# aelmiger/LINE-MOD-Pipeline

Hardware: AMD Instinct MI355X
Metric: detections/sec (higher is better)
Workload: dtype u8

## Files before the change

line-mod-pipeline_amd/csrc/lm_common.h:

```cpp
#pragma once
#include <stdint.h>

typedef uint8_t u8;
typedef uint16_t u16;
typedef uint32_t u32;
typedef uint64_t u64;

#define LM_SCAN_CHUNK 1008
#define LM_SCAN4_CHUNK 1016
#define LM_SCAN_FPAD 8
#define LM_SCANL_LDS_BYTES 163840
#define LM_SCANL_IMAGE_MAX 153600
#define LM_SCANL_TABLE_BYTES 2048
#define LM_SCANL_POS_BITS 15
#define LM_SORT_CAP 4096
#define LM_SORT_CHUNK 1024
#define LM_INLINE_MATCHES 2048
#define LM_DROPPED 0xFFFFFFFFu

#define PD_STRIP 16
#define CB_ROWS 2
#define CBS_STRIP 16
#define MX_WAVE_BYTES 128
#define CVT_ROWS 4
#define CG_STRIP 16
#define CT_W 32
#define CT_H 8
#define DT_W 64
#define DT_H 8
#define DM_ROWS 4
#ifndef DM_ROWS_BATCH
#define DM_ROWS_BATCH 16
#endif
#define LMK_MAX_LOADS 8

struct LmPhaseGrid { u32 nb[4]; int g[4]; };

struct LmLevelGeom {
    int w, h;
    int T;
    int W, H;
    int spread_only;
    int nibble;
    u32 wh;
    u32 ori_stride;
    u32 plane_ori;
    u32 mod_stride;
// ... 42 lines not shown
```

line-mod-pipeline_amd/csrc/lm_detector.hip:

```cpp
#include "lm_detector_impl.h"
#include "lm_median_counts.h"

namespace lmd {

thread_local std::string g_err;
int fail(int code, const std::string& msg) { g_err = msg; return code; }

bool any_lane_busy(const lm_detector* d) {
    for (const lm_detector::Lane& ln : d->lanes) if (ln.busy) return true;
    return false;
}

void free_device_bank(lm_detector* d) {
    for (auto* b : {&d->d_item_t, &d->d_item_chunk, &d->d_scan_off, &d->d_off1, &d->d_offn, &d->d_offs3, &d->d_offl, &d->d_offsl, &d->d_litem}) b->reset();
    for (auto* b : {&d->d_scan_P, &d->d_scan_n, &d->d_t_global, &d->d_t_class}) b->reset();
    d->items1.clear();
    for (int l = 0; l < LM_MAX_LEVELS; ++l) { d->d_ref_meta[l].reset(); d->d_ref_feat[l].reset(); }
}

int ensure_device(lm_detector* d) {
    if (d->dev_ready) {
        HIP_TRY(hipSetDevice(d->cfg.device));
        return LM_OK;
    }
// ... 102 lines not shown
    }
    d->luts_dirty = false;
    return LM_OK;
}

int ensure_bank(lm_detector* d) {
    if (!d->bank_dirty) return LM_OK;
    HIP_TRY(hipDeviceSynchronize());
    free_device_bank(d);
    std::string err;
    if (!lmh::build_device_bank(d->bank, d->cfg, d->geom, d->hb, d->scan_list_order, err)) return fail(LM_ERR_INVALID, err);
    HIP_TRY(upload_vec(d->d_item_t, d->hb.item_t));
    HIP_TRY(upload_vec(d->d_item_chunk, d->hb.item_chunk));
    HIP_TRY(upload_vec(d->d_scan_off, d->hb.scan_off));
    HIP_TRY(upload_vec(d->d_scan_P, d->hb.scan_P));
    HIP_TRY(upload_vec(d->d_scan_n, d->hb.scan_n));
    if (d->hb.fpad1) {
        HIP_TRY(upload_vec(d->d_off1, d->hb.off1));
        HIP_TRY(upload_vec(d->d_offn, d->hb.offn));
        HIP_TRY(upload_vec(d->d_offs3, d->hb.offs3));
    }
    if (d->hb.lds_ok) {
        HIP_TRY(upload_vec(d->d_offl, d->hb.offl));
        HIP_TRY(upload_vec(d->d_offsl, d->hb.offsl));
        HIP_TRY(upload_vec(d->d_litem, d->hb.lrec));
    }
    HIP_TRY(upload_vec(d->d_t_global, d->hb.t_global));
    HIP_TRY(upload_vec(d->d_t_class, d->hb.t_class));
    for (int l = 0; l + 1 < d->cfg.pyramid_levels; ++l) {
        HIP_TRY(upload_vec(d->d_ref_meta[l], d->hb.ref_meta[l]));
        HIP_TRY(upload_vec(d->d_ref_feat[l], d->hb.ref_feat[l]));
    }
    d->bank_dirty = false;
    return LM_OK;
}

int check_slots(lm_detector* d, int first, int n) {
    if (first < 0 || n < 0 || first + n > (int)d->slots.size()) return fail(LM_ERR_INVALID, "slot out of range");
    return LM_OK;
}

bool normal_lut_onehot(lm_detector* d) {
    if (d->lut_onehot < 0) {
        d->lut_onehot = 1;
        for (int i = 0; i < 8000; ++i) { const u8 v = d->normal_lut[i]; if (v & (v - 1)) { d->lut_onehot = 0; break; } }
    }
    return d->lut_onehot != 0;
}

int refuse_checked_slots(const lm_detector* d, int first, int n) {
    if (d->cc_inflight && d->cc_pending && first <= d->cc_hi && d->cc_lo < first + n) return fail(LM_ERR_INVALID, "slot is read by a colour check in flight: call lm_color_check_end first");
    if (d->dc_inflight && d->dc_pending && first <= d->dc_hi && d->dc_lo < first + n) return fail(LM_ERR_INVALID, "slot is read by depth counts in flight: call lm_depth_counts_end first");
    const int icp_slot = d->icp_slot.load();
    if (icp_slot >= first && icp_slot < first + n) return fail(LM_ERR_INVALID, "slot is read by an ICP refinement in flight");
    return LM_OK;
}

lmh::ScanInputs scan_inputs(const lm_detector* d, const lm_detector::Lane& ln) {
    const LmLevelGeom& g = d->geom[d->cfg.pyramid_levels - 1];
    lmh::ScanInputs in;
    in.form = d->scan_form; in.M = d->cfg.num_modalities;
    in.nibble = g.nibble != 0; in.planes = g.plane_ori != 0; in.lds_fits = lmh::lds_image_fits(g, in.M);
    in.bank_built = !d->bank_dirty;
    in.scanl_bank = d->hb.lds_ok && d->d_litem; in.scanl_device = d->scanl_lds;
    in.fpad1 = d->hb.fpad1; in.items1_by_L = d->hb.items1_by_L; in.items4 = (long long)d->hb.item_t.size();
    in.frame_stride = d->frame_stride; in.arena_bytes = g.arena_bytes;
// ... 246 lines not shown

static int refuse_scan(lmh::ScanPlan::Kind k) {
    if (k == lmh::ScanPlan::Mixed)
        return fail(LM_ERR_INVALID, "the slots were prepared by calls of different scan forms (some keep only the spread byte of the scanned level): match them apart or upload again");
    return fail(LM_ERR_HIP, "the slots keep only the spread byte of the scanned level and the bit-plane scan could not be set up for them: upload the frames again");
}

static bool ensure_surv_queue(lm_detector* d, lm_detector::Lane& ln) {
    DevBuf<unsigned long long>& q = ln.d_surv;
    if (!q) {
        if (q.alloc(16 + (size_t)d->surv_cap) != hipSuccess) (void)hipGetLastError();
        else if (hipMemsetAsync(q, 0, 16 * sizeof(unsigned long long), ln.stream) != hipSuccess) { q.reset(); (void)hipGetLastError(); }
        ln.surv_set = 0;
    }
    return q != nullptr;
}

static lmh::MatchInputs match_inputs(const lm_detector* d, const lm_detector::Lane& ln, int first, ItemRange r, int nslots, int variant) {
    const int L = d->cfg.pyramid_levels;
    const LmLevelGeom& g = d->geom[L - 1];
    lmh::MatchInputs in;
    in.scan = scan_inputs(d, ln);
    in.layouts = slot_layouts(d, first, nslots); in.nslots = nslots;
    in.n_items = r.n;
    in.n_litems = d->hb.lds_ok ? d->hb.lbegin[(size_t)r.t_hi] - d->hb.lbegin[(size_t)r.t_lo] : 0;
    in.T = g.T; in.wh = g.wh; in.ori_stride = g.ori_stride; in.nibble = g.nibble != 0;
    in.M = d->cfg.num_modalities; in.L = L;
    for (int l = 0; l < L; ++l) in.level_W[l] = d->geom[l].W;
    in.miss_delta = d->miss_delta;
    in.have_plan = ln.plan != nullptr; in.plan_stride_cap = d->plan_stride_cap;
    in.variant = variant;
    in.sort_split_mode = d->sort_split_mode; in.sort_long_score = d->sort_long_score;
    return in;
}

int make_scan_args(lm_detector* d, lm_detector::Lane& ln, int first, ItemRange r, int nslots, int variant, lmh::MatchPlan* plan, LmScanArgs* out) {
    const int L = d->cfg.pyramid_levels;
    const LmLevelGeom& g = d->geom[L - 1];
    lmh::MatchInputs in = match_inputs(d, ln, first, r, nslots, variant);
    const lm_detector::Items1* it = nullptr;
    if (const int L1 = lmh::match_scan1_lanes(in))
        if (ensure_items1(d, L1, &it) == LM_OK) {
            in.items1_L = L1; in.n_items1 = it->begin[(size_t)r.t_hi] - it->begin[(size_t)r.t_lo];
            in.have_queue = ensure_surv_queue(d, ln);
        }
    lmh::MatchPlan& p = *plan;
    lmh::plan_match(in, p);
    if (p.kind == lmh::ScanPlan::Mixed || p.kind == lmh::ScanPlan::NoBitPlaneForm) return refuse_scan(p.kind);
    LmScanArgs& a = *out;
    a = LmScanArgs();
    a.lm = d->lm(first, L - 1); a.lm_slot_stride = d->frame_stride;
    a.item_t = d->d_item_t; a.item_chunk = d->d_item_chunk; a.item_lo = r.lo; a.n_items = p.n_items;
    a.nibble = g.nibble; a.M = d->cfg.num_modalities; a.fpad = d->hb.fpad; a.W = g.W; a.T = g.T;
    a.scan_off = d->d_scan_off; a.scan_P = d->d_scan_P; a.scan_n = d->d_scan_n;
    a.raw_thr_by_n = ln.d_raw_thr;
    a.hdr = reinterpret_cast<LmDevHeader*>(d->aux(first, d->off_hdr));
    a.cand = reinterpret_cast<LmCand*>(d->aux(first, d->off_cand));
    a.aux_slot_stride = d->aux_stride; a.cand_cap = d->max_cand;
    a.stat = d->scan_stats ? d->d_scan_stat : nullptr;
    a.wgs_per_slot = p.wgs_per_slot; a.nslots = nslots;
    a.L1 = p.L1; a.G1 = p.G1; a.L1_rcp16 = p.L1_rcp16; a.delta_rcp16 = p.delta_rcp16; a.no_exact = p.no_exact; a.exact_spread = p.exact_spread ? 1 : 0;
    a.R = p.R; a.pb = p.pb; a.planes_off = p.planes_off; a.tbl_bytes = p.tbl_bytes; a.queue_cap = p.queue_cap; a.dbg = p.dbg;
    if (p.kind != lmh::ScanPlan::Scan4) { a.fpad1 = d->hb.fpad1; a.offs3 = d->d_offs3; a.resp_tab = d->d_resp_tab; }
    if (p.kind == lmh::ScanPlan::ScanL) {
        a.lds_form = 1;
        a.offl = d->d_offl; a.offsl = d->d_offsl; a.litem = d->d_litem; a.litem_lo = d->hb.lbegin[(size_t)r.t_lo]; a.n_litems = in.n_litems;
        a.mod_stride = g.mod_stride; a.plane_ori = g.plane_ori;
    } else if (p.kind == lmh::ScanPlan::Scan1) {
        a.off1 = d->d_off1; a.offn = d->d_offn;
        a.item_t = it->d_t; a.item_chunk = it->d_chunk; a.item_lo = it->begin[(size_t)r.t_lo];
        a.surv = p.queue ? ln.d_surv : nullptr; a.surv_cap = d->surv_cap; a.surv_set = ln.surv_set;
    }
    return LM_OK;
}

void launch_scan(lm_detector::Lane& ln, const lmh::MatchPlan& plan, LmScanArgs& a) {
    lmk_scan_run(ln.stream, plan, a, ln.d_surv);
    if (!plan.flip_surv_set) return;
    ln.surv_set ^= 1;
    a.surv_set = ln.surv_set;
}

static LmRefineArgs make_refine_args(lm_detector* d, const lm_detector::Lane& ln, int first, int n, int level, float threshold, const lmh::MatchPlan& p) {
    LmRefineArgs a;
    a.lm = d->lm(first, level); a.lm_slot_stride = d->frame_stride;
    a.g = d->geom[level];
    a.M = d->cfg.num_modalities;
    a.meta = d->d_ref_meta[level]; a.feats = d->d_ref_feat[level];
    a.sim_lut = d->d_sim_lut;
    a.hdr = reinterpret_cast<LmDevHeader*>(d->aux(first, d->off_hdr));
    a.cand = reinterpret_cast<LmCand*>(d->aux(first, d->off_cand));
    a.keys = reinterpret_cast<u64*>(d->aux(first, d->off_keys));
    a.aux_slot_stride = d->aux_stride;
    a.cand_cap = d->max_cand; a.match_cap = d->max_match;
    a.threshold = threshold;
    a.t_global = d->d_t_global; a.t_class = d->d_t_class;
    a.plan = p.refine_plan ? ln.plan : nullptr; a.plan_cap = p.plan_cap;
    a.blocks_per_slot = p.blocks_per_slot; a.nslots = n;
// ... 679 lines not shown
```

line-mod-pipeline_amd/csrc/lm_detector_impl.h:

```cpp
#pragma once
#include <hip/hip_runtime.h>

#include <algorithm>
#include <climits>
#include <cmath>
#include <cstdio>
#include <cstdlib>
#include <cstring>
#include <string>
#include <vector>
#include <memory>
#include <mutex>
#include <atomic>

#include "../../include/linemod_hip.h"
#include "lm_common.h"
#include "lm_extract.h"
#include <thread>

#include "lm_host.h"
#include "lm_yaml.h"
#include "lm_kernels.h"
#include "lm_comm.h"
#include "lm_own.h"
// ... 42 lines not shown
struct IcpState;
struct GenState;
struct EvalState;

}
using namespace lmd;

struct lm_detector {
    ~lm_detector();
    lm_config cfg;
    LmLevelGeom geom[LM_MAX_LEVELS];
    int lw[LM_MAX_LEVELS], lh[LM_MAX_LEVELS];
    u8 sim_lut[256];
    u8 normal_lut[8000];
    int lut_onehot = -1;
    bool normal_lut_substitute = true;
    lmh::Bank bank;

    bool dev_ready = false;
    bool dev_begun = false;
    struct Gather {
        DevBuf<int> d_cnt; DevBuf<LmOutMatch> d_rec;
        DevBuf<int> d_all_cnt; DevBuf<LmOutMatch> d_all_rec;
        PinnedBuf<int> h_all_cnt; PinnedBuf<LmOutMatch> h_all_rec;
        bool active = false;
        u32 cap_lane = 0;
    };
    struct Lane {
        Stream stream;
        Event ev[6];
        DevBuf<int> d_raw_thr;
        PinnedBuf<int> h_raw_thr;
        float raw_thr_for = -1.0f;
        bool created = false, busy = false, timed = false;
        Event ev_done;
        Event blocking_ev;
        Event mask_done;
        int first = 0, n = 0;
        std::vector<int> classes;
        unsigned long long waited_seq[LM_NCOPY] = {};
        DevBuf<unsigned long long> d_surv;
        int surv_set = 0;
        u32* plan = nullptr;
        Gather gather;
        std::unique_ptr<LmComm> comm;
    };
    Lane lanes[LM_NLANES];
    Stream copy_stream[LM_NCOPY];
    unsigned long long up_seq_next[LM_NCOPY], up_seq_done[LM_NCOPY];
    int n_copy_streams = LM_NCOPY;
    int stage_chunks = 1;
    std::vector<Slot> slots;
    PinnedBuf<LmIngestDesc> h_ingest;
    DevBuf<LmIngestDesc> d_ingest;
    Event ev_ingest_src;
    bool reg_on = false, reg_rays_dirty = false;
    lm_registration_desc reg = {};
    std::vector<float> reg_rays;
    DevBuf<float> d_reg_rays;
    DevBuf<u32> d_reg_z[LM_NCOPY];
    bool rect_on = false, rect_map_dirty = false;
    lm_rectification_desc rect = {};
    std::vector<int32_t> rect_map;
    DevBuf<int32_t> d_rect_map;
    DevBuf<u8> frame_arena;
    size_t frame_stride = 0;
// ... 18 lines not shown
    int comm_recs_per_frame = 0;
    DevBuf<double> d_red;
    int batch_phases = 2;
    int scan_list_order = 3;
    int sort_split_mode = 2;
    int sort_long_score = 0;
    int work_weight_by_pixels = 1;
    int phase_max_slots = 15;
    DevBuf<u8> aux_arena;
    size_t aux_stride = 0;
    size_t off_hdr = 0, off_cand = 0, off_keys = 0, off_out = 0;
    PinnedBuf<u8> host_blocks;
    size_t host_stride = 0;
    DevBuf<u32> d_plan;
    int plan_stride_cap = 0;
    DevBuf<u64> d_resp_tab;
    int miss_delta = 1;
    DevBuf<u32> d_sim_lut;
    DevBuf<u8> d_normal_lut;
    bool luts_dirty = true;
    bool bank_dirty = true;
    lmh::DeviceBankHost hb;
    DevBuf<u32> d_item_t, d_item_chunk;
    DevBuf<u32> d_scan_off; DevBuf<int> d_scan_P, d_scan_n;
    DevBuf<int> d_t_global, d_t_class;
    DevBuf<u32> d_off1, d_offn;
    struct Items1 { int L = 0; DevBuf<u32> d_t, d_chunk; std::vector<int> begin; };
    std::vector<Items1> items1;
    int scan_form = 0;
    float scan1_min_threshold = 50.0f;
    long long cnt_scan1_launches = 0; int last_scan1_lanes = 0;
    DevBuf<u32> d_offs3;
    DevBuf<u32> d_offl, d_offsl, d_litem;
    DevBuf<unsigned long long> d_refine_stat;
    int scanl_min_slots = 24;
    int scanl_R = 0;
    bool scanl_lds = false;
    u32 surv_cap = 1u << 20;
    DevBuf<LmRefMeta> d_ref_meta[LM_MAX_LEVELS];
    DevBuf<LmRefFeat> d_ref_feat[LM_MAX_LEVELS];
    DevBuf<u8> d_scratch;
    u32 max_cand = 0, max_match = 0;
    int scan_variant = 0;
    bool scan_stats = false;
    DevBuf<unsigned long long> d_scan_stat;
    bool profiling = false;
    double prof_us[4] = {0, 0, 0, 0};
    double prof_scan_bytes = 0;
    long long prof_launches = 0, prof_frames = 0;
    long long prof_exch_fallbacks = 0;
    double prof_exch_us = 0; long long prof_exch_launches = 0;
    long long cnt_preprocess_frames = 0, cnt_scan_launches = 0, cnt_refine_launches = 0, cnt_sort_launches = 0;

    u8* bgr(int slot, int l) const { return frame_arena + (size_t)slot * frame_stride + off_bgr[l]; }
    u16* depth(int slot) const { return reinterpret_cast<u16*>(frame_arena + (size_t)slot * frame_stride + off_depth); }
    u8* quant(int slot, int l, int m) const { return frame_arena + (size_t)slot * frame_stride + off_quant[l][m]; }
    u8* lm(int slot, int l) const { return frame_arena + (size_t)slot * frame_stride + off_lm[l]; }
    u8* cscratch(int slot, int l = 0) const { return frame_arena + (size_t)slot * frame_stride + (l == 0 ? off_cscratch : off_cscratch1); }
    u8* dscratch(int slot) const { return frame_arena + (size_t)slot * frame_stride + off_dscratch; }
    u8* aux(int slot, size_t off) const { return aux_arena + (size_t)slot * aux_stride + off; }
    LmHostBlock* host_block(int slot) const { return reinterpret_cast<LmHostBlock*>(host_blocks + (size_t)slot * host_stride); }
};

namespace lmd {

struct ItemRange { int lo, n; int t_lo, t_hi; };
// ... 62 lines not shown
```

line-mod-pipeline_amd/csrc/lm_host.cpp:

```cpp
#include "lm_host.h"
#if defined(__x86_64__)
#include <immintrin.h>
#endif

#include <algorithm>
#include <atomic>
#include <cassert>
#include <cmath>
#include <cstdio>
#include <cstdlib>
#include <cstring>

namespace lmh {

int Bank::find(const std::string& id) const {
    for (size_t i = 0; i < classes.size(); ++i)
        if (classes[i].id == id) return (int)i;
    return -1;
}

int Bank::add_pyramid(const std::string& id, TemplatePyramid&& tp) {
    int ci = find(id);
    if (ci < 0) { classes.push_back(ClassEntry{id, {}}); ci = (int)classes.size() - 1; }
    classes[ci].pyramids.push_back(std::move(tp));
// ... 220 lines not shown
                mt.width = tp[(size_t)l * M].width;
                mt.height = tp[(size_t)l * M].height;
                for (int m = 0; m < M; ++m) {
                    const Template& t = tp[(size_t)l * M + m];
                    mt.nfeat_total += (int)t.features.size();
                    mt.start[m] = (u32)out.ref_feat[l].size();
                    mt.count[m] = (u32)t.features.size();
                    for (const lm_feature& f : t.features) {
                        LmRefFeat rf;
                        rf.off = ((u32)m * g.mod_stride + (u32)((f.y % g.T) * g.T + (f.x % g.T)) * g.wh +
                                  (u32)(f.y / g.T) * g.W + (u32)(f.x / g.T)) |
                                 ((u32)f.label << 29);
                        if ((u64)m * g.mod_stride + (u64)((f.y % g.T) * g.T + (f.x % g.T)) * g.wh + (u64)(f.y / g.T) * g.W +
                                (u64)(f.x / g.T) >= (1ull << 29)) { err = "feature too far outside the frame"; return false; }
                        rf.x = (int16_t)f.x; rf.y = (int16_t)f.y;
                        out.ref_feat[l].push_back(rf);
                    }
                }
                out.ref_meta[l].push_back(mt);
            }
        }
        out.class_t_hi[ci] = (int)out.t_global.size();
        out.class_item_hi[ci] = (int)out.item_t.size();
    }
    if (out.lds_ok) {
        out.lbegin.push_back((int)out.litem.size());
        if (out.t_global.size() >= (1u << (32 - LM_SCANL_POS_BITS)) || out.litem.empty()) out.lds_ok = false;
    }
    if (out.lds_ok) {
        schedule_lds_lists(out);
        out.lrec.assign(out.litem.size() * 4u, 0u);
        for (size_t i = 0; i < out.litem.size(); ++i) {
            const u32 it = out.litem[i];
            out.lrec[4 * i] = it;
            if (it != 0xFFFFFFFFu) { out.lrec[4 * i + 1] = (u32)out.scan_n[it >> 8]; out.lrec[4 * i + 2] = (u32)out.scan_P[it >> 8]; }
        }
    }
    return true;
}

void schedule_lds_lists(DeviceBankHost& out) {
    const size_t nt = out.t_global.size();
    const int fp = out.fpad1;
    auto residue = [](u32 e) { return (int)(((e >> 8) >> 2) & 3u); };
    std::vector<u32> tmp((size_t)fp);
    std::vector<char> used((size_t)fp);
    for (size_t t = 0; t < nt; ++t) {
        const int lb = out.lbegin[t], le = out.lbegin[t + 1];
        int last = le;
        while (last > lb && out.litem[(size_t)last - 1] == 0xFFFFFFFFu) --last;
        if (last <= lb) continue;
        const int g_first = lb / 32;
        std::vector<size_t> nb;
        for (size_t p = t; p-- > 0 && nb.size() < 8;) {
            int pl = out.lbegin[p + 1];
            while (pl > out.lbegin[p] && out.litem[(size_t)pl - 1] == 0xFFFFFFFFu) --pl;
            if (pl <= out.lbegin[p]) continue;
            if ((pl - 1) / 32 < g_first) break;
            nb.push_back(p);
        }
        if (nb.empty()) continue;
        u32* list = out.offl.data() + t * (size_t)fp;
        const int cnt = out.scan_n[t];
        const int nreal = std::min(fp, ((cnt >> 8) & 0xFF) + ((cnt >> 16) & 0xFF));
        std::fill(used.begin(), used.end(), 0);
        for (int k = 0; k < nreal; ++k) {
            bool taken[4] = {false, false, false, false};
            for (size_t p : nb) taken[residue(out.offl[p * (size_t)fp + (size_t)k])] = true;
            int pick = -1, first = -1;
            for (int q = 0; q < nreal; ++q) {
                if (used[(size_t)q]) continue;
// ... 719 lines not shown
```

line-mod-pipeline_amd/csrc/lm_host.h:

```cpp
#pragma once
#include <string>
#include <vector>

#include "../../include/linemod_hip.h"
#include "lm_common.h"

namespace lmh {

struct Template {
    int width = 0, height = 0, pyramid_level = 0;
    std::vector<lm_feature> features;
};
typedef std::vector<Template> TemplatePyramid;

struct ClassEntry {
    std::string id;
    std::vector<TemplatePyramid> pyramids;
};

struct Bank {
    std::vector<ClassEntry> classes;
    int find(const std::string& id) const;
    int add_class(const std::string& id, int n_templates, const lm_template_desc* descs, const lm_feature* features,
                  int levels, int modalities, std::string& err);
    int add_pyramid(const std::string& id, TemplatePyramid&& tp);
};

bool check_template_pyramid(const TemplatePyramid& tp, int levels, int modalities, std::string& err);
bool check_modality_params(const lm_config& cfg, std::string& err);

struct DeviceBankHost {
    int fpad = LM_SCAN_FPAD;
    std::vector<int> t_global, t_class;
    std::vector<u32> scan_off;
    std::vector<int> scan_P, scan_n;
    std::vector<u32> item_t, item_chunk;
    std::vector<int> class_item_lo, class_item_hi;
    std::vector<int> class_t_lo, class_t_hi;
    std::vector<double> class_alg_bytes;
    std::vector<double> class_load_bytes;
    std::vector<LmRefMeta> ref_meta[LM_MAX_LEVELS];
    std::vector<LmRefFeat> ref_feat[LM_MAX_LEVELS];
    int fpad1 = 0;
    std::vector<u32> off1, offn, offs3;
    long long items1_by_L[65] = {};
    bool lds_ok = false;
    std::vector<u32> offl;
    std::vector<u32> offsl;
    std::vector<u32> litem;
    std::vector<u32> lrec;
    std::vector<int> lbegin;
};
void build_items1(const DeviceBankHost& hb, int L, std::vector<u32>& item_t, std::vector<u32>& item_chunk, std::vector<int>& begin);
bool lds_image_fits(const LmLevelGeom& g, int M);

enum class Layout : unsigned char {
    Responses,
    ResponsesAndPlanes,
    SpreadAndPlanes,
};
inline unsigned layout_bit(Layout l) { return 1u << (unsigned)l; }
inline bool layouts_mixed(unsigned held) {
    return (held & layout_bit(Layout::SpreadAndPlanes)) && held != layout_bit(Layout::SpreadAndPlanes);
}

struct ScanInputs {
    int form = 0;
    int M = 1;
    bool nibble = false, planes = false;
    bool lds_fits = false;
    bool bank_built = false;
    bool scanl_bank = false;
    bool scanl_device = false;
    int fpad1 = 0;
    const long long* items1_by_L = nullptr;
    long long items4 = 0;
    size_t frame_stride = 0;
    u32 arena_bytes = 0;
    float threshold = -1.0f;
    float scan1_min_threshold = 50.0f;
    int scanl_min_slots = 24;
    int scanl_R = 0;
};

Layout plan_layout(const ScanInputs& in, int n);

struct ScanPlan {
// ... 217 lines not shown
```

line-mod-pipeline_amd/csrc/lm_k_scan.hip:

```cpp
#include "lm_dev.h"
#include "lm_host.h"

namespace {

template <int UNROLL, bool XCD_MAP>
__global__ __launch_bounds__(256) void k_scan(LmScanArgs a) {
    const int lane = threadIdx.x & 63;
    u32 slot, wg;
    if (XCD_MAP) {
        const u32 G = (u32)a.wgs_per_slot, B = (u32)a.nslots;
        const u32 b = blockIdx.x, x = b & 7u, k = b >> 3;
        if ((B & 7u) == 0) { slot = x + 8u * (k / G); wg = k % G; }
        else { const u32 r = 8u / B; slot = x % B; wg = k * r + x / B; }
        if (wg >= G || slot >= B) return;
    } else {
        slot = blockIdx.z; wg = blockIdx.x;
    }
    const int wave = __builtin_amdgcn_readfirstlane((int)((wg * 256u + threadIdx.x) >> 6));
    if (wave >= a.n_items) return;
    const u32 ti = a.item_t[a.item_lo + wave];
    const u32 chunk = a.item_chunk[a.item_lo + wave];
    const int P = a.scan_P[ti];
    const int n = a.scan_n[ti] & 0xFF;
    const int thr = a.raw_thr_by_n[n];
// ... 527 lines not shown
            n0 = __builtin_amdgcn_raw_buffer_load_b128(rs_off, voff, nf, 0);
            n1 = __builtin_amdgcn_raw_buffer_load_b128(rs_off, voff, nf + 16u, 0);
            const u32 e[8] = {e0[0], e0[1], e0[2], e0[3], e1[0], e1[1], e1[2], e1[3]};
            u32 v[8][5];
#pragma unroll
            for (int k = 0; k < 8; ++k) {
                const lds_u32_t* p = (const lds_u32_t*)(unsigned long)((e[k] + unit_add) >> 8);
                v[k][0] = p[0]; v[k][1] = p[1]; v[k][2] = p[2]; v[k][3] = p[3];
            }
#pragma unroll
            for (int k = 0; k < 8; ++k) v[k][4] = next_lane(v[k][0]) & keep5;
            u32 x[4][8];
#pragma unroll
            for (int k = 0; k < 8; ++k) {
#pragma unroll
                for (int q = 0; q < 4; ++q) x[q][k] = __builtin_amdgcn_alignbit(v[k][q + 1], v[k][q], e[k]);
            }
#pragma unroll
            for (int q = 0; q < 4; ++q) bs_level<0, 8, TOP>(c[q], x[q]);
        }
        if (f + 8 > first_test && f + 8 < Fw) {
            const unsigned long long left = __ballot((c[0][TOP] & c[1][TOP] & c[2][TOP] & c[3][TOP]) != 0xFFFFFFFFu) & alive;
            if (!left) pruned = true;
            else alive = left;
        }
    }
#pragma unroll
    for (int q = 0; q < 4; ++q) flags[q] = c[q][TOP];
    f_out = f;
    return pruned;
}

__device__ __forceinline__ u32 tabs_at(const u8* lds, u32 img, u32 sv, u32 ori) { return lds[img + sv * 8u + ori]; }
__global__ __launch_bounds__(1024) void k_scanl(LmScanArgs a) {
    extern __shared__ u32x4 scanl_lds[];
    u8* lds = reinterpret_cast<u8*>(scanl_lds);
    const int tid = (int)threadIdx.x, lane = tid & 63, wave = tid >> 6;
    u32 slot, r;
    {
        const u32 R = (u32)a.R, B = (u32)a.nslots, b = blockIdx.x;
        if ((B & 7u) == 0) { const u32 x = b & 7u, k = b >> 3; slot = x + 8u * (k / R); r = k - (k / R) * R; }
        else { slot = b / R; r = b - slot * R; }
    }
    if (slot >= (u32)a.nslots) return;
    const u8* arena = a.lm + (size_t)slot * a.lm_slot_stride;
    const u32 IMG = (u32)a.M * 8u * a.pb;
    u32* qcount = reinterpret_cast<u32*>(lds + IMG + a.tbl_bytes);
    const int* thr_tab = reinterpret_cast<const int*>(qcount + 4);
    u32* queue = qcount + 4 + 128;
    const u32 n_w = ((u32)a.n_litems + 63u) >> 6;
    const unsigned long long tm0 = __builtin_readcyclecounter();
    const u32 n_share = n_w > r ? (n_w - r + (u32)a.R - 1u) / (u32)a.R : 0u;
    const u32x4 no_item = {0xFFFFFFFFu, 0u, 0u, 0u};
    auto item_at = [&](u32 j) -> u32x4 {
        const u32 idx = (r + (u32)a.R * j) * 64u + (u32)lane;
        return (j < n_share && idx < (u32)a.n_litems) ? reinterpret_cast<const u32x4*>(a.litem)[(size_t)a.litem_lo + idx] : no_item;
    };
    u32 j_cur = (u32)wave;
    u32x4 rec_cur = item_at(j_cur);
    {
        const u32 per = a.pb >> 4, np = (u32)a.M * 8u, wpp = 16u / np;
        const u32 pl = (u32)wave % np, part = (u32)wave / np, m = pl >> 3, o = pl & 7u;
        const u8* src = arena + (size_t)m * a.mod_stride + a.planes_off + (size_t)o * a.plane_ori;
        u32x4* dst = scanl_lds + (size_t)pl * per;
        const u32 stride = 64u * wpp;
        if (part < wpp && a.dbg != 3) {
            const u32 rot = (r * per) / (u32)a.R;
            for (u32 k0 = (u32)lane + 64u * part; k0 < per; k0 += 8u * stride) {
                u32x4 t[8];
#pragma unroll
                for (int q = 0; q < 8; ++q) { const u32 k = k0 + (u32)q * stride, kk = k + rot < per ? k + rot : k + rot - per; t[q] = k < per ? *reinterpret_cast<const u32x4*>(src + 16u * kk) : u32x4{0, 0, 0, 0}; }
#pragma unroll
                for (int q = 0; q < 8; ++q) { const u32 k = k0 + (u32)q * stride, kk = k + rot < per ? k + rot : k + rot - per; if (k < per) dst[kk] = t[q]; }
            }
        }
        for (u32 i = (u32)tid; i < (a.tbl_bytes >> 2); i += 1024u) reinterpret_cast<u32*>(lds + IMG)[i] = 0u;
        if (tid < 128) const_cast<int*>(thr_tab)[tid] = a.raw_thr_by_n[tid];
        if (tid == 0) { qcount[0] = 0u; qcount[1] = 16u; }
    }
    __syncthreads();
    const unsigned long long tm1 = __builtin_readcyclecounter();
    const __amdgpu_buffer_rsrc_t rs_off = __builtin_amdgcn_make_buffer_rsrc(const_cast<u32*>(a.offl), 0, 0x7FFFFFFF, 0x00020000);
    const u32 lds_base = (u32)(unsigned long)(__attribute__((address_space(3))) u32x4*)scanl_lds;
    unsigned long long st_f = 0, st_F = 0, st_l = 0, st_s = 0;
    for (; j_cur < n_share; ) {
        const u32 it = rec_cur[0];
        const int cnt = (int)rec_cur[1], P = (int)rec_cur[2];
        j_cur = (u32)__builtin_amdgcn_readfirstlane((int)(lane == 0 ? atomicAdd(qcount + 1, 1u) : 0u));
        rec_cur = item_at(j_cur);
        const bool has = it != 0xFFFFFFFFu;
        const u32 ti = has ? it >> 8 : 0u, unit = has ? it & 255u : 0u;
        const int n = cnt & 0xFF;
        const int F = ((cnt >> 8) & 0xFF) + ((cnt >> 16) & 0xFF);
        const int thr = thr_tab[n & 127];
        const int K0 = 4 * F - thr - 1;
        int mmax = K0 >= 0 ? (int)(((u32)K0 * a.delta_rcp16) >> 16) : 0;
        if (mmax > 127) mmax = 127;
        const u32 pre = (u32)(127 - mmax);
        const int j0 = (int)unit * 128;
        int valid = (has && K0 >= 0) ? P - j0 : 0;
        valid = valid < 0 ? 0 : (valid > 128 ? 128 : valid);
        unsigned long long alive = __ballot(valid > 0);
        if (!alive) continue;
        const int Fw = __builtin_amdgcn_readfirstlane((int)wave_max_u32(valid > 0 ? (u32)F : 0u));
        const int mm_hi = __builtin_amdgcn_readfirstlane((int)wave_max_u32(valid > 0 ? (u32)mmax : 0u));
        const int first_test = 127 - __builtin_amdgcn_readfirstlane((int)wave_max_u32(valid > 0 ? pre : 0u));
        const u32 voff = ti * (u32)a.fpad1 * 4u;
        const u32 unit_add = (unit * 16u + lds_base) << 8;
        u32 keep5 = (j0 + 128 >= P || lane == 63) ? 0u : 0xFFFFFFFFu;
        asm volatile("" : "+v"(keep5));
        u32 flags[4];
        bool pruned;
        int f;
        if (mm_hi <= 31) pruned = scanl_rounds<5>(rs_off, voff, unit_add, keep5, (u32)(31 - mmax), valid, Fw, first_test, alive, flags, f);
        else pruned = scanl_rounds<7>(rs_off, voff, unit_add, keep5, pre, valid, Fw, first_test, alive, flags, f);
        st_l += (unsigned long long)f * 64ull;
        st_f += (unsigned long long)(f < Fw ? f : Fw); st_F += (unsigned long long)Fw;
        u32 h[4];
#pragma unroll
        for (int q = 0; q < 4; ++q) h[q] = (pruned || !((alive >> lane) & 1ull)) ? 0u : ~flags[q];
        const u32 nh = (u32)(__popc(h[0]) + __popc(h[1]) + __popc(h[2]) + __popc(h[3]));
        if (nh && !a.no_exact) {
            const u32 at = atomicAdd(qcount, nh);
            u32 fit = at >= a.queue_cap ? 0u : min(nh, a.queue_cap - at);
            st_s += fit;
            u32* q = queue + at;
            const u32 hi = ti << LM_SCANL_POS_BITS;
#pragma unroll
            for (int k = 0; k < 4; ++k)
                for (; h[k] && fit; --fit) { const int b = __ffs((int)h[k]) - 1; *q++ = hi | (u32)(j0 + 32 * k + b); h[k] &= h[k] - 1u; }
        }
        unsigned long long hl = a.no_exact ? 0ull : __ballot((h[0] | h[1] | h[2] | h[3]) != 0u);
        while (hl) {
            const int src = __ffsll((long long)hl) - 1;
            const u32 w0 = (u32)__builtin_amdgcn_readlane((int)h[0], src), w1 = (u32)__builtin_amdgcn_readlane((int)h[1], src);
            const u32 w2 = (u32)__builtin_amdgcn_readlane((int)h[2], src), w3 = (u32)__builtin_amdgcn_readlane((int)h[3], src);
            const int q = w0 ? 0 : (w1 ? 1 : (w2 ? 2 : 3));
            const u32 wq = w0 ? w0 : (w1 ? w1 : (w2 ? w2 : w3));
            const int b = __ffs((int)wq) - 1;
            const int j = __builtin_amdgcn_readlane(j0, src) + 32 * q + b;
            const u32 sti = (u32)__builtin_amdgcn_readlane((int)ti, src);
            const int sF = __builtin_amdgcn_readlane(F, src), sn = __builtin_amdgcn_readlane(n, src), sthr = __builtin_amdgcn_readlane(thr, src);
            if (lane == src) {
#pragma unroll
                for (int k = 0; k < 4; ++k) h[k] = (k == q) ? (h[k] & ~(1u << b)) : h[k];
            }
            const u32* o3 = a.offs3 + (size_t)sti * a.fpad1;
            u32 vv = 0;
            if (lane < sF) { const u32 on = o3[lane]; vv = (u32)((a.resp_tab[arena[(on & 0x1FFFFFFFu) + (u32)j]] >> (8u * (on >> 29))) & 0xFFu); }
            if (lane + 64 < sF) { const u32 on = o3[lane + 64]; vv += (u32)((a.resp_tab[arena[(on & 0x1FFFFFFFu) + (u32)j]] >> (8u * (on >> 29))) & 0xFFu); }
            const int raw = (int)wave_sum_u32(vv);
            st_s += (lane == 0) ? 1u : 0u;
            if (raw > sthr && lane == 0) scanl_emit(a, slot, sti, j, raw, sn);
            hl = __ballot((h[0] | h[1] | h[2] | h[3]) != 0u);
        }
    }
    const unsigned long long tm2 = __builtin_readcyclecounter();
    if (a.stat && a.dbg != 7) {
        unsigned long long sv = st_s;
#pragma unroll
        for (int sft = 32; sft >= 1; sft >>= 1) sv += (unsigned long long)__shfl_xor((long long)sv, sft, 64);
        if (lane == 0) {
            atomicAdd(&a.stat[4 * (blockIdx.x & 1023u)], st_f);
            atomicAdd(&a.stat[4 * (blockIdx.x & 1023u) + 1], st_F);
            atomicAdd(&a.stat[4 * (blockIdx.x & 1023u) + 2], st_l);
            atomicAdd(&a.stat[4 * (blockIdx.x & 1023u) + 3], sv);
        }
    }
    if (a.no_exact) return;
    __syncthreads();
    const unsigned long long tm3 = __builtin_readcyclecounter();
    const u32 qn = min(*qcount, a.queue_cap);
    if (qn == 0) return;
    const u32 F_MASK = 0x1FFFFFFFu;
    u32x4 ent[16];
    u32 e_cur = 0xFFFFFFFFu;
    int cn_cur = 0;
    auto request = [&](u32 i, int half) {
        e_cur = i < qn ? queue[i] : 0xFFFFFFFFu;
        const u32 ti = e_cur >> LM_SCANL_POS_BITS;
        if (e_cur != 0xFFFFFFFFu) {
            cn_cur = a.scan_n[ti];
            const u32x4* of = reinterpret_cast<const u32x4*>(a.offsl + (size_t)ti * a.fpad1) + 16 * half;
#pragma unroll
            for (int q = 0; q < 16; ++q) ent[q] = (64 * half + 4 * q < a.fpad1) ? of[q] : u32x4{0, 0, 0, 0};
        }
    };
    auto partial = [&](int F, u32 j, int half) -> int {
        int raw = 0;
#pragma unroll
        for (int q = 0; q < 16; ++q) {
#pragma unroll
            for (int c4 = 0; c4 < 4; ++c4) {
                const u32 o = ent[q][c4];
                if (64 * half + 4 * q + c4 < F) raw += (int)tabs_at(lds, IMG, (u32)lds[(o & F_MASK) + j], o >> 29);
            }
        }
        return raw;
    };
    u32 i0 = (u32)tid;
    request(i0, 0);
    {
        const u32 per = (a.pb * 8u) >> 4;
        for (int m = 0; m < (a.dbg == 2 ? 0 : a.M); ++m) {
            const u8* src = arena + (size_t)m * a.mod_stride;
            u32x4* dst = scanl_lds + (size_t)m * per;
            const u32 rot = (r * per) / (u32)a.R;
            for (u32 k0 = (u32)tid; k0 < per; k0 += 4u * 1024u) {
                u32x4 t[4];
#pragma unroll
                for (int q = 0; q < 4; ++q) { const u32 k = k0 + (u32)q * 1024u, kk = k + rot < per ? k + rot : k + rot - per; t[q] = k < per ? *reinterpret_cast<const u32x4*>(src + 16u * kk) : u32x4{0, 0, 0, 0}; }
#pragma unroll
                for (int q = 0; q < 4; ++q) { const u32 k = k0 + (u32)q * 1024u, kk = k + rot < per ? k + rot : k + rot - per; if (k < per) dst[kk] = t[q]; }
            }
        }
        if (tid < 256) reinterpret_cast<u64*>(lds + IMG)[tid] = a.resp_tab[tid];
    }
    __syncthreads();
    const unsigned long long tm4 = __builtin_readcyclecounter();
    if (a.dbg == 1) return;
    for (; i0 < qn; ) {
        const u32 e = e_cur;
        const u32 ti = e >> LM_SCANL_POS_BITS, j = e & ((1u << LM_SCANL_POS_BITS) - 1u);
        const int n = cn_cur & 0xFF;
        const int F = ((cn_cur >> 8) & 0xFF) + ((cn_cur >> 16) & 0xFF);
        int raw = partial(F, j, 0);
        if (F > 64) { request(i0, 1); raw += partial(F, j, 1); }
        if (raw > thr_tab[n & 127]) scanl_emit(a, slot, ti, (int)j, raw, n);
        i0 += 1024u;
        if (i0 < qn) request(i0, 0);
    }
    if (a.stat && a.dbg == 7 && lane == 0) {
        const unsigned long long tm5 = __builtin_readcyclecounter();
        atomicAdd(&a.stat[4 * (blockIdx.x & 1023u)], tm1 - tm0);
        atomicAdd(&a.stat[4 * (blockIdx.x & 1023u) + 1], tm2 - tm1);
        atomicAdd(&a.stat[4 * (blockIdx.x & 1023u) + 2], (tm3 - tm2) + ((tm4 - tm3) << 32));
        atomicAdd(&a.stat[4 * (blockIdx.x & 1023u) + 3], tm5 - tm4);
    }
}


}

bool lmk_scanl_raise_lds() {
    if (hipFuncSetAttribute(reinterpret_cast<const void*>(k_scanl), hipFuncAttributeMaxDynamicSharedMemorySize, LM_SCANL_LDS_BYTES) == hipSuccess) return true;
    (void)hipGetLastError();
    return false;
}

void lmk_scan_run(hipStream_t s, const lmh::MatchPlan& plan, const LmScanArgs& a, unsigned long long* queue) {
    using K = lmh::MatchKernel;
    for (int i = 0; i < plan.scan_end; ++i) {
        const lmh::MatchStep& st = plan.step[i];
        const dim3 grid(st.gx, st.gy, st.gz), block(st.block);
#define RUN(...) hipLaunchKernelGGL((__VA_ARGS__), grid, block, st.lds, s, a); break
        switch (st.k) {
            case K::SurvReset: (void)hipMemsetAsync(queue, 0, 16 * sizeof(unsigned long long), s); break;
            case K::Scan8X: RUN(k_scan<8, true>);
            case K::Scan4X: RUN(k_scan<4, true>);
            case K::Scan2X: RUN(k_scan<2, true>);
            case K::Scan8: RUN(k_scan<8, false>);
            case K::Scan4: RUN(k_scan<4, false>);
            case K::Scan2: RUN(k_scan<2, false>);
            case K::Scan4_6_P0: RUN(k_scan4<6, true, 0>);
            case K::Scan4_6_P1: RUN(k_scan4<6, true, 1>);
            case K::Scan4_6_P2: RUN(k_scan4<6, true, 2>);
            case K::Scan4_12_P0: RUN(k_scan4<12, true, 0>);
            case K::Scan4_12_P1: RUN(k_scan4<12, true, 1>);
            case K::Scan4_12_P2: RUN(k_scan4<12, true, 2>);
            case K::Scan4_3_P0: RUN(k_scan4<3, true, 0>);
            case K::Scan4_3_P1: RUN(k_scan4<3, true, 1>);
            case K::Scan4_3_P2: RUN(k_scan4<3, true, 2>);
            case K::Scan4NoShift: RUN(k_scan4<6, true, 0, true>);
            case K::Scan1: RUN(k_scan1);
            case K::Scan1Exact: RUN(k_scan1_exact);
            case K::ScanL: RUN(k_scanl);
            default: break;
        }
#undef RUN
    }
}
```

line-mod-pipeline_amd/csrc/lm_kernels.h:

```cpp
#pragma once
#include <hip/hip_runtime.h>
#include "../../include/linemod_hip.h"
#include "lm_common.h"
#include "lm_ingest_check.h"
#include "lm_register.h"
#include "lm_rectify.h"

struct LmPreArgs {
    int L;
    int w[LM_MAX_LEVELS], h[LM_MAX_LEVELS], T[LM_MAX_LEVELS], mode[LM_MAX_LEVELS];
    u32 ori_stride[LM_MAX_LEVELS];
    u8* bgr[LM_MAX_LEVELS];
    u8* cs[LM_MAX_LEVELS];
    float* mag[LM_MAX_LEVELS];
    u8* quant[LM_MAX_LEVELS][2];
    u8* lm[LM_MAX_LEVELS][2];
    const u16* depth; u8* ds;
    float weak_threshold; int dist_thr, diff_thr;
    const u8* normal_lut; const u64* resp_tab;
    u32 planes;
    size_t slot_stride; int nslots;
};
namespace lmh { struct PrePlan; struct MatchPlan; }
size_t lmk_color_scratch_bytes(int w, int h);
// ... 90 lines not shown
    const u32* item_chunk;
    int item_lo, n_items;
    int nibble;
    const u32* scan_off;
    const int* scan_P;
    const int* scan_n;
    int M, fpad;
    const int* raw_thr_by_n;
    int W, T;
    LmDevHeader* hdr;
    LmCand* cand;
    size_t aux_slot_stride;
    u32 cand_cap;
    unsigned long long* stat;
    int wgs_per_slot, nslots;
    int L1, G1;
    u32 L1_rcp16;
    u32 delta_rcp16;
    const u32* off1;
    const u32* offn;
    int fpad1;
    int no_exact;
    unsigned long long* surv;
    u32 surv_cap;
    int surv_set;
    int exact_spread;
    const u32* offs3;
    const u64* resp_tab;
    int lds_form, R;
    const u32* offl;
    const u32* offsl;
    const u32* litem;
    int litem_lo, n_litems;
    u32 pb;
    u32 mod_stride, planes_off, plane_ori;
    u32 tbl_bytes;
    u32 queue_cap;
    int dbg;
};
#define LM_SCAN_VARIANT_SETTABLE (0x3F | 0x100)
void lmk_scan_run(hipStream_t s, const lmh::MatchPlan& plan, const LmScanArgs& a, unsigned long long* queue);
bool lmk_scanl_raise_lds();

struct LmRefineArgs {
    const u8* lm;
    size_t lm_slot_stride;
    LmLevelGeom g;
    int M;
    const LmRefMeta* meta;
    const LmRefFeat* feats;
    const u32* sim_lut;
    LmDevHeader* hdr;
    LmCand* cand;
    u64* keys;
    size_t aux_slot_stride;
    u32 cand_cap;
    u32 match_cap;
    float threshold;
    const int* t_global;
    const int* t_class;
    const u32* plan;
    int plan_cap;
    int blocks_per_slot, nslots;
    unsigned long long* stat;
};
struct LmSortArgs {
// ... 113 lines not shown
```

Measured before the change: 202,700.

## Precompute per-wave and per-lane ScanL pruning tables on host

Moves the per-item threshold, mmax, valid-count and wave-wide max reductions of the ScanL kernel into a host-built table, rebuilt only when the threshold, template bank or miss delta change. Item records are repacked so voff, keep5 and the emit base come precomputed, and whole waves with no live items are skipped early. The stats and cycle-counter code is compiled out through a template parameter when stats are off. The cost is extra table loads per item and a host rebuild with a stream sync whenever parameters change.

Result: no change. 203,500, median of 6 (+0.4%).

```diff
diff --git a/line-mod-pipeline_amd/csrc/lm_common.h b/line-mod-pipeline_amd/csrc/lm_common.h
--- a/line-mod-pipeline_amd/csrc/lm_common.h
+++ b/line-mod-pipeline_amd/csrc/lm_common.h
@@ -13,6 +13,8 @@
 #define LM_SCANL_IMAGE_MAX 153600
 #define LM_SCANL_TABLE_BYTES 2048
 #define LM_SCANL_POS_BITS 15
+#define LM_SCANL_REC_KEEP5 0x80000000u
+#define LM_SCANL_WT_LIVE 0x80000000u
 #define LM_SORT_CAP 4096
 #define LM_SORT_CHUNK 1024
 #define LM_INLINE_MATCHES 2048
diff --git a/line-mod-pipeline_amd/csrc/lm_detector.hip b/line-mod-pipeline_amd/csrc/lm_detector.hip
--- a/line-mod-pipeline_amd/csrc/lm_detector.hip
+++ b/line-mod-pipeline_amd/csrc/lm_detector.hip
@@ -158,6 +158,7 @@
         HIP_TRY(upload_vec(d->d_ref_feat[l], d->hb.ref_feat[l]));
     }
     d->bank_dirty = false;
+    d->bank_gen += 1;
     return LM_OK;
 }
 
@@ -470,6 +471,20 @@
     in.variant = variant;
     in.sort_split_mode = d->sort_split_mode; in.sort_long_score = d->sort_long_score;
     return in;
+}
+
+static int ensure_scanl_table(lm_detector* d, lm_detector::Lane& ln) {
+    if (ln.d_wtab && ln.wtab_thr == ln.raw_thr_for && ln.wtab_bank == d->bank_gen && ln.wtab_delta == d->miss_delta) return LM_OK;
+    HIP_TRY(hipStreamSynchronize(ln.stream));
+    std::vector<u32> tab;
+    lmh::build_scanl_wave_table(d->hb, ln.h_raw_thr, d->miss_delta, tab);
+    const size_t n = std::max<size_t>(tab.size(), 1);
+    HIP_TRY(ln.d_wtab.grow(n));
+    HIP_TRY(ln.h_wtab.grow(n));
+    std::copy(tab.begin(), tab.end(), ln.h_wtab.get());
+    HIP_TRY(hipMemcpyAsync(ln.d_wtab, ln.h_wtab, tab.size() * sizeof(u32), hipMemcpyHostToDevice, ln.stream));
+    ln.wtab_thr = ln.raw_thr_for; ln.wtab_bank = d->bank_gen; ln.wtab_delta = d->miss_delta;
+    return LM_OK;
 }
 
 int make_scan_args(lm_detector* d, lm_detector::Lane& ln, int first, ItemRange r, int nslots, int variant, lmh::MatchPlan* plan, LmScanArgs* out) {
@@ -502,6 +517,8 @@
     if (p.kind != lmh::ScanPlan::Scan4) { a.fpad1 = d->hb.fpad1; a.offs3 = d->d_offs3; a.resp_tab = d->d_resp_tab; }
     if (p.kind == lmh::ScanPlan::ScanL) {
         a.lds_form = 1;
+        if (int rc = ensure_scanl_table(d, ln)) return rc;
+        a.wtab = ln.d_wtab; a.ltab = ln.d_wtab.get() + (d->hb.lrec.size() / 4u + 63u) / 64u;
         a.offl = d->d_offl; a.offsl = d->d_offsl; a.litem = d->d_litem; a.litem_lo = d->hb.lbegin[(size_t)r.t_lo]; a.n_litems = in.n_litems;
         a.mod_stride = g.mod_stride; a.plane_ori = g.plane_ori;
     } else if (p.kind == lmh::ScanPlan::Scan1) {
diff --git a/line-mod-pipeline_amd/csrc/lm_detector_impl.h b/line-mod-pipeline_amd/csrc/lm_detector_impl.h
--- a/line-mod-pipeline_amd/csrc/lm_detector_impl.h
+++ b/line-mod-pipeline_amd/csrc/lm_detector_impl.h
@@ -98,6 +98,11 @@
         DevBuf<int> d_raw_thr;
         PinnedBuf<int> h_raw_thr;
         float raw_thr_for = -1.0f;
+        DevBuf<u32> d_wtab;
+        PinnedBuf<u32> h_wtab;
+        float wtab_thr = -1.0f;
+        unsigned long long wtab_bank = 0;
+        int wtab_delta = 0;
         bool created = false, busy = false, timed = false;
         Event ev_done;
         Event blocking_ev;
@@ -182,6 +187,7 @@
     long long cnt_scan1_launches = 0; int last_scan1_lanes = 0;
     DevBuf<u32> d_offs3;
     DevBuf<u32> d_offl, d_offsl, d_litem;
+    unsigned long long bank_gen = 0;
     DevBuf<unsigned long long> d_refine_stat;
     int scanl_min_slots = 24;
     int scanl_R = 0;
diff --git a/line-mod-pipeline_amd/csrc/lm_host.cpp b/line-mod-pipeline_amd/csrc/lm_host.cpp
--- a/line-mod-pipeline_amd/csrc/lm_host.cpp
+++ b/line-mod-pipeline_amd/csrc/lm_host.cpp
@@ -276,11 +276,41 @@
         out.lrec.assign(out.litem.size() * 4u, 0u);
         for (size_t i = 0; i < out.litem.size(); ++i) {
             const u32 it = out.litem[i];
+            if (it == 0xFFFFFFFFu) continue;
+            const u32 ti = it >> 8, unit = it & 255u;
+            const int cnt = out.scan_n[ti], P = out.scan_P[ti], j0 = (int)unit * 128;
+            const u32 n = (u32)cnt & 0xFFu, F = (u32)(((cnt >> 8) & 0xFF) + ((cnt >> 16) & 0xFF));
+            const u32 valid = (u32)std::max(0, std::min(128, P - j0));
+            const bool keep5 = j0 + 128 < P && (i & 63u) != 63u;
             out.lrec[4 * i] = it;
-            if (it != 0xFFFFFFFFu) { out.lrec[4 * i + 1] = (u32)out.scan_n[it >> 8]; out.lrec[4 * i + 2] = (u32)out.scan_P[it >> 8]; }
+            out.lrec[4 * i + 1] = n | (F << 8) | (valid << 16) | (keep5 ? LM_SCANL_REC_KEEP5 : 0u);
+            out.lrec[4 * i + 2] = ti * (u32)out.fpad1 * 4u;
+            out.lrec[4 * i + 3] = (ti << LM_SCANL_POS_BITS) | (u32)j0;
         }
     }
     return true;
+}
+
+void build_scanl_wave_table(const DeviceBankHost& hb, const int* raw_thr_by_n, int miss_delta, std::vector<u32>& out) {
+    const size_t n_items = hb.lrec.size() / 4u;
+    const u32 delta_rcp16 = (65536u + (u32)miss_delta - 1u) / (u32)miss_delta;
+    const size_t n_waves = (n_items + 63u) / 64u;
+    out.assign(n_waves + n_items, 0u);
+    for (size_t w = 0; w < n_waves; ++w) {
+        u32 Fw = 0, mm_hi = 0, mm_lo = 127;
+        bool live = false;
+        for (size_t i = 64u * w; i < std::min(n_items, 64u * w + 64u); ++i) {
+            const u32 rc = hb.lrec[4 * i + 1];
+            const int n = (int)(rc & 0xFFu), F = (int)((rc >> 8) & 0xFFu), valid = (int)((rc >> 16) & 0xFFu);
+            const int K0 = 4 * F - raw_thr_by_n[n & 127] - 1;
+            if (valid <= 0 || K0 < 0) continue;
+            const u32 mmax = std::min<u32>(((u32)K0 * delta_rcp16) >> 16, 127u);
+            out[n_waves + i] = mmax | ((u32)valid << 8);
+            live = true;
+            Fw = std::max(Fw, (u32)F); mm_hi = std::max(mm_hi, mmax); mm_lo = std::min(mm_lo, mmax);
+        }
+        if (live) out[w] = Fw | (mm_hi << 8) | (mm_lo << 16) | LM_SCANL_WT_LIVE;
+    }
 }
 
 void schedule_lds_lists(DeviceBankHost& out) {
diff --git a/line-mod-pipeline_amd/csrc/lm_host.h b/line-mod-pipeline_amd/csrc/lm_host.h
--- a/line-mod-pipeline_amd/csrc/lm_host.h
+++ b/line-mod-pipeline_amd/csrc/lm_host.h
@@ -53,6 +53,7 @@
 };
 void build_items1(const DeviceBankHost& hb, int L, std::vector<u32>& item_t, std::vector<u32>& item_chunk, std::vector<int>& begin);
 bool lds_image_fits(const LmLevelGeom& g, int M);
+void build_scanl_wave_table(const DeviceBankHost& hb, const int* raw_thr_by_n, int miss_delta, std::vector<u32>& out);
 
 enum class Layout : unsigned char {
     Responses,
diff --git a/line-mod-pipeline_amd/csrc/lm_k_scan.hip b/line-mod-pipeline_amd/csrc/lm_k_scan.hip
--- a/line-mod-pipeline_amd/csrc/lm_k_scan.hip
+++ b/line-mod-pipeline_amd/csrc/lm_k_scan.hip
@@ -583,6 +583,7 @@
 }
 
 __device__ __forceinline__ u32 tabs_at(const u8* lds, u32 img, u32 sv, u32 ori) { return lds[img + sv * 8u + ori]; }
+template <bool STATS>
 __global__ __launch_bounds__(1024) void k_scanl(LmScanArgs a) {
     extern __shared__ u32x4 scanl_lds[];
     u8* lds = reinterpret_cast<u8*>(scanl_lds);
@@ -600,15 +601,24 @@
     const int* thr_tab = reinterpret_cast<const int*>(qcount + 4);
     u32* queue = qcount + 4 + 128;
     const u32 n_w = ((u32)a.n_litems + 63u) >> 6;
-    const unsigned long long tm0 = __builtin_readcyclecounter();
+    unsigned long long tm0 = 0, tm1 = 0, tm2 = 0, tm3 = 0, tm4 = 0;
+    if constexpr (STATS) tm0 = __builtin_readcyclecounter();
     const u32 n_share = n_w > r ? (n_w - r + (u32)a.R - 1u) / (u32)a.R : 0u;
-    const u32x4 no_item = {0xFFFFFFFFu, 0u, 0u, 0u};
+    const u32x4 no_item = {0u, 0u, 0u, 0u};
     auto item_at = [&](u32 j) -> u32x4 {
         const u32 idx = (r + (u32)a.R * j) * 64u + (u32)lane;
         return (j < n_share && idx < (u32)a.n_litems) ? reinterpret_cast<const u32x4*>(a.litem)[(size_t)a.litem_lo + idx] : no_item;
     };
-    u32 j_cur = (u32)wave;
+    u32 vzero = 0u;
+    asm volatile("" : "+v"(vzero));
+    auto wave_at = [&](u32 j) -> u32 { return j < n_share ? a.wtab[((u32)a.litem_lo >> 6) + r + (u32)a.R * j + vzero] : 0u; };
+    auto lane_at = [&](u32 j) -> u32 {
+        const u32 idx = (r + (u32)a.R * j) * 64u + (u32)lane;
+        return (j < n_share && idx < (u32)a.n_litems) ? a.ltab[(size_t)a.litem_lo + idx] : 0u;
+    };
+    u32 j_cur = (u32)__builtin_amdgcn_readfirstlane(wave);
     u32x4 rec_cur = item_at(j_cur);
+    u32 wt_cur = wave_at(j_cur), lt_cur = lane_at(j_cur);
     {
         const u32 per = a.pb >> 4, np = (u32)a.M * 8u, wpp = 16u / np;
         const u32 pl = (u32)wave % np, part = (u32)wave / np, m = pl >> 3, o = pl & 7u;
@@ -630,58 +640,52 @@
         if (tid == 0) { qcount[0] = 0u; qcount[1] = 16u; }
     }
     __syncthreads();
-    const unsigned long long tm1 = __builtin_readcyclecounter();
+    if constexpr (STATS) tm1 = __builtin_readcyclecounter();
     const __amdgpu_buffer_rsrc_t rs_off = __builtin_amdgcn_make_buffer_rsrc(const_cast<u32*>(a.offl), 0, 0x7FFFFFFF, 0x00020000);
     const u32 lds_base = (u32)(unsigned long)(__attribute__((address_space(3))) u32x4*)scanl_lds;
     unsigned long long st_f = 0, st_F = 0, st_l = 0, st_s = 0;
     for (; j_cur < n_share; ) {
-        const u32 it = rec_cur[0];
-        const int cnt = (int)rec_cur[1], P = (int)rec_cur[2];
+        const u32 it = rec_cur[0], rc = rec_cur[1], voff = rec_cur[2], ebase = rec_cur[3];
+        const u32 wt = (u32)__builtin_amdgcn_readfirstlane((int)wt_cur), lt = lt_cur;
         j_cur = (u32)__builtin_amdgcn_readfirstlane((int)(lane == 0 ? atomicAdd(qcount + 1, 1u) : 0u));
         rec_cur = item_at(j_cur);
-        const bool has = it != 0xFFFFFFFFu;
-        const u32 ti = has ? it >> 8 : 0u, unit = has ? it & 255u : 0u;
-        const int n = cnt & 0xFF;
-        const int F = ((cnt >> 8) & 0xFF) + ((cnt >> 16) & 0xFF);
-        const int thr = thr_tab[n & 127];
-        const int K0 = 4 * F - thr - 1;
-        int mmax = K0 >= 0 ? (int)(((u32)K0 * a.delta_rcp16) >> 16) : 0;
-        if (mmax > 127) mmax = 127;
+        wt_cur = wave_at(j_cur); lt_cur = lane_at(j_cur);
+        if (!(wt & LM_SCANL_WT_LIVE)) continue;
+        const u32 ti = it >> 8, unit = it & 255u;
+        const int mmax = (int)(lt & 0xFFu), valid = (int)(lt >> 8);
         const u32 pre = (u32)(127 - mmax);
         const int j0 = (int)unit * 128;
-        int valid = (has && K0 >= 0) ? P - j0 : 0;
-        valid = valid < 0 ? 0 : (valid > 128 ? 128 : valid);
         unsigned long long alive = __ballot(valid > 0);
-        if (!alive) continue;
-        const int Fw = __builtin_amdgcn_readfirstlane((int)wave_max_u32(valid > 0 ? (u32)F : 0u));
-        const int mm_hi = __builtin_amdgcn_readfirstlane((int)wave_max_u32(valid > 0 ? (u32)mmax : 0u));
-        const int first_test = 127 - __builtin_amdgcn_readfirstlane((int)wave_max_u32(valid > 0 ? pre : 0u));
-        const u32 voff = ti * (u32)a.fpad1 * 4u;
+        const int Fw = (int)(wt & 0xFFu), mm_hi = (int)((wt >> 8) & 0xFFu), first_test = (int)((wt >> 16) & 0xFFu);
         const u32 unit_add = (unit * 16u + lds_base) << 8;
-        u32 keep5 = (j0 + 128 >= P || lane == 63) ? 0u : 0xFFFFFFFFu;
+        u32 keep5 = (u32)((int)rc >> 31);
         asm volatile("" : "+v"(keep5));
         u32 flags[4];
         bool pruned;
         int f;
         if (mm_hi <= 31) pruned = scanl_rounds<5>(rs_off, voff, unit_add, keep5, (u32)(31 - mmax), valid, Fw, first_test, alive, flags, f);
         else pruned = scanl_rounds<7>(rs_off, voff, unit_add, keep5, pre, valid, Fw, first_test, alive, flags, f);
-        st_l += (unsigned long long)f * 64ull;
-        st_f += (unsigned long long)(f < Fw ? f : Fw); st_F += (unsigned long long)Fw;
+        if constexpr (STATS) {
+            st_l += (unsigned long long)f * 64ull;
+            st_f += (unsigned long long)(f < Fw ? f : Fw); st_F += (unsigned long long)Fw;
+        }
+        if (pruned) continue;
         u32 h[4];
 #pragma unroll
-        for (int q = 0; q < 4; ++q) h[q] = (pruned || !((alive >> lane) & 1ull)) ? 0u : ~flags[q];
+        for (int q = 0; q < 4; ++q) h[q] = !((alive >> lane) & 1ull) ? 0u : ~flags[q];
         const u32 nh = (u32)(__popc(h[0]) + __popc(h[1]) + __popc(h[2]) + __popc(h[3]));
         if (nh && !a.no_exact) {
             const u32 at = atomicAdd(qcount, nh);
             u32 fit = at >= a.queue_cap ? 0u : min(nh, a.queue_cap - at);
-            st_s += fit;
+            if constexpr (STATS) st_s += fit;
             u32* q = queue + at;
-            const u32 hi = ti << LM_SCANL_POS_BITS;
 #pragma unroll
             for (int k = 0; k < 4; ++k)
-                for (; h[k] && fit; --fit) { const int b = __ffs((int)h[k]) - 1; *q++ = hi | (u32)(j0 + 32 * k + b); h[k] &= h[k] - 1u; }
+                for (; h[k] && fit; --fit) { const int b = __ffs((int)h[k]) - 1; *q++ = ebase + (u32)(32 * k + b); h[k] &= h[k] - 1u; }
         }
         unsigned long long hl = a.no_exact ? 0ull : __ballot((h[0] | h[1] | h[2] | h[3]) != 0u);
+        if (!hl) continue;
+        const int n = (int)(rc & 0xFFu), F = (int)((rc >> 8) & 0xFFu), thr = thr_tab[n & 127];
         while (hl) {
             const int src = __ffsll((long long)hl) - 1;
             const u32 w0 = (u32)__builtin_amdgcn_readlane((int)h[0], src), w1 = (u32)__builtin_amdgcn_readlane((int)h[1], src);
@@ -701,13 +705,13 @@
             if (lane < sF) { const u32 on = o3[lane]; vv = (u32)((a.resp_tab[arena[(on & 0x1FFFFFFFu) + (u32)j]] >> (8u * (on >> 29))) & 0xFFu); }
             if (lane + 64 < sF) { const u32 on = o3[lane + 64]; vv += (u32)((a.resp_tab[arena[(on & 0x1FFFFFFFu) + (u32)j]] >> (8u * (on >> 29))) & 0xFFu); }
             const int raw = (int)wave_sum_u32(vv);
-            st_s += (lane == 0) ? 1u : 0u;
+            if constexpr (STATS) st_s += (lane == 0) ? 1u : 0u;
             if (raw > sthr && lane == 0) scanl_emit(a, slot, sti, j, raw, sn);
             hl = __ballot((h[0] | h[1] | h[2] | h[3]) != 0u);
         }
     }
-    const unsigned long long tm2 = __builtin_readcyclecounter();
-    if (a.stat && a.dbg != 7) {
+    if constexpr (STATS) tm2 = __builtin_readcyclecounter();
+    if (STATS && a.stat && a.dbg != 7) {
         unsigned long long sv = st_s;
 #pragma unroll
         for (int sft = 32; sft >= 1; sft >>= 1) sv += (unsigned long long)__shfl_xor((long long)sv, sft, 64);
@@ -720,7 +724,7 @@
     }
     if (a.no_exact) return;
     __syncthreads();
-    const unsigned long long tm3 = __builtin_readcyclecounter();
+    if constexpr (STATS) tm3 = __builtin_readcyclecounter();
     const u32 qn = min(*qcount, a.queue_cap);
     if (qn == 0) return;
     const u32 F_MASK = 0x1FFFFFFFu;
@@ -768,7 +772,7 @@
         if (tid < 256) reinterpret_cast<u64*>(lds + IMG)[tid] = a.resp_tab[tid];
     }
     __syncthreads();
-    const unsigned long long tm4 = __builtin_readcyclecounter();
+    if constexpr (STATS) tm4 = __builtin_readcyclecounter();
     if (a.dbg == 1) return;
     for (; i0 < qn; ) {
         const u32 e = e_cur;
@@ -781,7 +785,7 @@
         i0 += 1024u;
         if (i0 < qn) request(i0, 0);
     }
-    if (a.stat && a.dbg == 7 && lane == 0) {
+    if (STATS && a.stat && a.dbg == 7 && lane == 0) {
         const unsigned long long tm5 = __builtin_readcyclecounter();
         atomicAdd(&a.stat[4 * (blockIdx.x & 1023u)], tm1 - tm0);
         atomicAdd(&a.stat[4 * (blockIdx.x & 1023u) + 1], tm2 - tm1);
@@ -794,7 +798,8 @@
 }
 
 bool lmk_scanl_raise_lds() {
-    if (hipFuncSetAttribute(reinterpret_cast<const void*>(k_scanl), hipFuncAttributeMaxDynamicSharedMemorySize, LM_SCANL_LDS_BYTES) == hipSuccess) return true;
+    if (hipFuncSetAttribute(reinterpret_cast<const void*>(k_scanl<false>), hipFuncAttributeMaxDynamicSharedMemorySize, LM_SCANL_LDS_BYTES) == hipSuccess &&
+        hipFuncSetAttribute(reinterpret_cast<const void*>(k_scanl<true>), hipFuncAttributeMaxDynamicSharedMemorySize, LM_SCANL_LDS_BYTES) == hipSuccess) return true;
     (void)hipGetLastError();
     return false;
 }
@@ -825,7 +830,7 @@
             case K::Scan4NoShift: RUN(k_scan4<6, true, 0, true>);
             case K::Scan1: RUN(k_scan1);
             case K::Scan1Exact: RUN(k_scan1_exact);
-            case K::ScanL: RUN(k_scanl);
+            case K::ScanL: if (a.stat) { RUN(k_scanl<true>); } else { RUN(k_scanl<false>); }
             default: break;
         }
 #undef RUN
diff --git a/line-mod-pipeline_amd/csrc/lm_kernels.h b/line-mod-pipeline_amd/csrc/lm_kernels.h
--- a/line-mod-pipeline_amd/csrc/lm_kernels.h
+++ b/line-mod-pipeline_amd/csrc/lm_kernels.h
@@ -146,6 +146,8 @@
     const u32* offsl;
     const u32* litem;
     int litem_lo, n_litems;
+    const u32* wtab;
+    const u32* ltab;
     u32 pb;
     u32 mod_stride, planes_off, plane_ori;
     u32 tbl_bytes;
```
